# adlternative/adlsm-tree

Measured on AMD Instinct MI355X. Metric: Mkeys/s bloom-filter build (device-resident), 16B keys, bits/key=10, higher is better.
Workload: dtype u32; 1 GPU; 10M x 16B keys, bits_per_key=10, one filter per GPU; keys_per_gpu=10000000, key_bytes=16, bits_per_key=10, filters_per_gpu=1, parallelism=whole filters per GPU x1, no data-path collective

## Files before the change

adlsm-tree_amd/csrc/bloom_build.hip:

```cpp
#include <hip/hip_ext.h>
#include <hip/hip_runtime.h>
#include <stdint.h>
#include <stdlib.h>
#include <string.h>

#include <algorithm>
#include <atomic>
#include <cmath>
#include <mutex>
#include <type_traits>
#include <vector>

#include "bloom_common.hpp"
#include "probe_server.hpp"

using namespace adl_dev;

namespace {

constexpr uint32_t kLdsWordsPerCu = 40960;
constexpr int kKptMax = 8;
constexpr int kBlockB = 1024;
constexpr int kDepthB = 8;
constexpr int kSegBatch = 2048;
// ... 316 lines not shown
        for (uint32_t win = 0; win < nwin; ++win) {
          const uint64_t wb = A0 + (uint64_t)win * S;
          const uint64_t we = min(wb + wcap, B1);
          const uint32_t nv = (uint32_t)((we - wb) >> 4);
          const uint4 *src = reinterpret_cast<const uint4 *>(keys.keys + wb);
          for (uint32_t v = tid; v < nv; v += BLOCK) stage4[v] = src[v];
          const uint32_t rem = (uint32_t)(we - wb) & 15u;
          if (rem && (uint32_t)tid < rem)
            reinterpret_cast<uint8_t *>(lpos)[nv * 16 + tid] = keys.keys[wb + nv * 16 + tid];
          __syncthreads();
          STAMP(6);
          const uint32_t wlo = win * S;
#pragma unroll
          for (int i = 0; i < KPT; ++i) {
            if (ks0[i] - wlo < S) {
              hash_lds(lpos, ks0[i] - wlo, klen[i], h1[i], h2[i]);
              pending &= ~(1u << i);
            }
          }
          __syncthreads();
          STAMP(7);
        }
#pragma unroll
        for (int i = 0; i < KPT; ++i)
          if (pending & (1u << i)) keys.hash(kb + kidx[i], h1[i], h2[i]);
      } else {
#pragma unroll
        for (int i = 0; i < KPT; ++i) {
          h1[i] = h2[i] = 0;
          if (slot_pos(i) < cnt) keys.hash(d.key_begin + first + kidx[i], h1[i], h2[i]);
        }
      }
    } else {
#pragma unroll
      for (int i = 0; i < KPT; ++i) {
        h1[i] = h2[i] = 0;
        if (slot_pos(i) < cnt) {
          if constexpr (PF) hash16(cur[i].raw, h1[i], h2[i]);
          else keys.hash(d.key_begin + first + kidx[i], h1[i], h2[i]);
        }
      }
    }
    uint32_t live = 0;
#pragma unroll
    for (int i = 0; i < KPT; ++i) {
      if (slot_pos(i) < cnt) {
        const uint32_t ki = first + kidx[i];
        if (!(a.dedup && ki > 0 && keys.same_as_prev(d.key_begin + ki))) live |= 1u << i;
      }
    }
    __syncthreads();
    STAMP(1);

    constexpr int KR = KFIX > 0 ? KFIX : 1;
    uint32_t pos[KPT][KR];
#pragma unroll
    for (int i = 0; i < KPT; ++i) {
      if (live & (1u << i)) {
        if constexpr (KFIX > 0) {
#pragma unroll
          for (int j = 0; j < KFIX; ++j) {
            pos[i][j] = fastmod(h1[i] + (uint32_t)j * h2[i], mod);
            atomicAdd(&hist[pos[i][j] >> TL], 1u);
          }
        } else {
          for (uint32_t j = 0; j < k; ++j) {
            const uint32_t p = fastmod(h1[i] + j * h2[i], mod);
            atomicAdd(&hist[p >> TL], 1u);
          }
        }
      }
    }
    __syncthreads();
    STAMP(2);

    const uint32_t total = block_excl_scan_array_1b<BLOCK>(hist, T + 1, scratch);

    uint32_t *tab = table_ws + d.table_base;
    for (uint32_t t = tid; t <= T; t += BLOCK) tab[(uint64_t)t * d.chunks + w] = hist[t];
    __syncthreads();
    STAMP(3);

#pragma unroll
    for (int i = 0; i < KPT; ++i) {
      if (live & (1u << i)) {
        if constexpr (KFIX > 0) {
          uint32_t slot_l[KFIX];
#pragma unroll
          for (int j = 0; j < KFIX; ++j) slot_l[j] = atomicAdd(&hist[pos[i][j] >> TL], 1u);
#pragma unroll
          for (int j = 0; j < KFIX; ++j) lpos[slot_l[j]] = pos[i][j] & tmask;
        } else {
          for (uint32_t j = 0; j < k; ++j) {
            const uint32_t p = fastmod(h1[i] + j * h2[i], mod);
            const uint32_t slot_l = atomicAdd(&hist[p >> TL], 1u);
            lpos[slot_l] = p & tmask;
          }
        }
      }
    }
    __syncthreads();
    STAMP(4);

    for (uint32_t i = tid; i <= T; i += BLOCK) hist[i] = 0;
    uint32_t *dst = pos_ws + d.pos_base + (uint64_t)w * a.cap;
    const uint32_t nvec = total >> 2;
    const uint4 *src4 = reinterpret_cast<const uint4 *>(lpos);
    uint4 *dst4 = reinterpret_cast<uint4 *>(dst);
    for (uint32_t i = tid; i < nvec; i += BLOCK) dst4[i] = src4[i];
    for (uint32_t i = (nvec << 2) + tid; i < total; i += BLOCK) dst[i] = lpos[i];
    STAMP(5);

    if constexpr (PF) {
#pragma unroll
      for (int i = 0; i < KPT; ++i) cur[i] = nxt[i];
    }
  }
  STAMP_FLUSH(0);
}

#ifndef ADL_HV_BLOCK
#define ADL_HV_BLOCK 256
#endif
constexpr int kHvBlock = ADL_HV_BLOCK;
constexpr uint32_t kHvBins = 512;
template <uint32_t S>
constexpr uint32_t hv_stage_bytes() {
  return S * 48;
}

template <uint32_t S>
constexpr size_t hv_lds_bytes() {
  return kHvBins * 4 + S * 4 + S * 2 + hv_stage_bytes<S>() + 16;
}

template <uint32_t S, bool DT>
__global__ __launch_bounds__(kHvBlock) void hash_var_kernel(BuildArgs a, KeysVar keys, uint2 *__restrict__ hp,
                                                            uint32_t total_sc, FilterTable ft) {
  extern __shared__ __attribute__((aligned(16))) uint32_t lds[];
  uint32_t *bins = lds;
  uint32_t *s_rel = lds + kHvBins;
  uint16_t *s_len = reinterpret_cast<uint16_t *>(s_rel + S);
  uint32_t *stage = reinterpret_cast<uint32_t *>(s_len + S);
  constexpr int KPT = S / kHvBlock;
  constexpr uint32_t NW = kHvBlock / kWave;
  const int tid = threadIdx.x, lane = tid & (kWave - 1), wave = tid / kWave;
  const uint32_t sc = blockIdx.x;
  if (sc >= total_sc) return;
  STAMP_DECL
  const auto &d = Filt<DT>::at(a, ft, Filt<DT>::of_run(a, ft, sc));
  const uint32_t first = (sc - d.sc_base) * S;
  const uint32_t cnt = min(S, d.n - first);
  const uint64_t kb = d.key_begin + first;
  const uint64_t base16 = keys.offs[kb] & ~15ull;
  const uint64_t end = keys.offs[kb + cnt];
  constexpr uint32_t kStage = hv_stage_bytes<S>();
  static_assert(kStage % (16 * kHvBlock) == 0, "the staging loads cover kStage in whole rounds of 16 B per thread");
  const uint32_t sbytes = (uint32_t)min((end - base16 + 15) & ~15ull, (uint64_t)kStage);

  constexpr int VPT = kStage / 16 / kHvBlock;
  const uint32_t nv = sbytes / 16;
  for (uint32_t i = tid; i < kHvBins; i += kHvBlock) bins[i] = 0;
  uint64_t o0[KPT], o1[KPT];
#pragma unroll
  for (int i = 0; i < KPT; ++i) {
    const uint32_t idx = min((uint32_t)(tid + i * kHvBlock), cnt - 1u);
    o0[i] = keys.offs[kb + idx];
    o1[i] = keys.offs[kb + idx + 1];
  }
  u32x4_t v[VPT];
  if (nv) {
    const u32x4_t *src = reinterpret_cast<const u32x4_t *>(keys.keys + base16);
#pragma unroll
    for (int i = 0; i < VPT; ++i) v[i] = src[min((uint32_t)(tid + i * kHvBlock), nv - 1u)];
  }
  __syncthreads();
  STAMP(0);
  uint32_t rk[KPT];
#pragma unroll
  for (int i = 0; i < KPT; ++i) {
    rk[i] = ~0u;
    if (tid + i * kHvBlock < cnt) {
      const uint32_t c = (uint32_t)min(o1[i] - o0[i], (uint64_t)(kHvBins - 1));
      rk[i] = (atomicAdd(&bins[c], 1u) << 9) | c;
    }
  }
  {
    u32x4_t *dst = reinterpret_cast<u32x4_t *>(stage);
#pragma unroll
    for (int i = 0; i < VPT; ++i)
      if (tid + i * kHvBlock < nv) dst[tid + i * kHvBlock] = v[i];
  }
  __syncthreads();
  STAMP(1);
  if (wave == 0) {
    constexpr int PER = kHvBins / kWave;
    uint32_t bv[PER], t = 0;
#pragma unroll
    for (int j = 0; j < PER; ++j) bv[j] = bins[lane * PER + j], t += bv[j];
    uint32_t run = wave_incl_scan(t, lane) - t;
#pragma unroll
    for (int j = 0; j < PER; ++j) bins[lane * PER + j] = run, run += bv[j];
  }
  __syncthreads();
  STAMP(2);
#pragma unroll
  for (int i = 0; i < KPT; ++i) {
    if (rk[i] != ~0u) {
      const uint32_t slot = bins[rk[i] & (kHvBins - 1)] + (rk[i] >> 9);
      const uint64_t len = o1[i] - o0[i];
      const bool near = len < 0xffffu && o0[i] - base16 < 0xffffffffull;
      s_rel[slot] = near ? (uint32_t)(o0[i] - base16) : tid + i * kHvBlock;
      s_len[slot] = near ? (uint16_t)len : (uint16_t)0xffffu;
    }
  }
  __syncthreads();
  STAMP(3);

  const uint32_t groups = (cnt + kWave - 1) / kWave;
  uint2 *out = hp + (uint64_t)d.chunk_base * a.C + first;
  for (uint32_t gi = wave; gi < groups; gi += NW) {
    const uint32_t g = groups - 1 - gi;
    const uint32_t s = g * kWave + lane;
    if (s >= cnt) continue;
    uint32_t len = s_len[s];
    const uint32_t r = s_rel[s];
    uint32_t h1, h2;
#ifdef ADL_BLOOM_STAMPS
    if (a.exp & 16) {
      out[s] = make_uint2(r, len | 1u);
      continue;
    }
#endif
    if (len < 0xffffu && (uint64_t)r + len <= sbytes) {
      hash_lds(stage, r, len, h1, h2);
    } else {
      uint64_t k0 = base16 + r;
      if (len == 0xffffu) {
        k0 = keys.offs[kb + r];
        len = (uint32_t)(keys.offs[kb + r + 1] - k0);
      }
      hash_bytes(keys.keys + k0, len, kSeed1, kSeed2, h1, h2);
    }
    out[s] = make_uint2(h1, h2);
  }
  STAMP(4);
  STAMP_FLUSH(2);
}

struct Src16 {
  const uint4 *keys;
  using Raw = uint4;
  __device__ __forceinline__ Raw load(const FilterDesc &d, uint32_t chunk, uint32_t first, uint32_t idx) const {
    return load_nt(keys + d.key_begin + first + idx);
  }
  __device__ static __forceinline__ void hash(const Raw &r, uint32_t &h1, uint32_t &h2) { hash16(r, h1, h2); }
};

typedef uint32_t u32x2_t __attribute__((ext_vector_type(2)));
struct SrcH {
  const uint2 *h;
  uint32_t C;
  using Raw = uint2;
  __device__ __forceinline__ Raw load(const FilterDesc &, uint32_t chunk, uint32_t, uint32_t idx) const {
    const u32x2_t v = __builtin_nontemporal_load(reinterpret_cast<const u32x2_t *>(h + (uint64_t)chunk * C + idx));
    return make_uint2(v.x, v.y);
  }
  __device__ static __forceinline__ void hash(const Raw &r, uint32_t &h1, uint32_t &h2) {
    h1 = r.x;
    h2 = r.y;
  }
};

template <int BLOCK, int K, class Src, bool DT, bool CL = false, bool DYN = false>
__global__ __launch_bounds__(BLOCK) kPassARegs void bloom_bin16_kernel(BuildArgs a, Src keys,
                                                              uint32_t *__restrict__ pos_ws,
                                                              uint32_t *__restrict__ table_ws,
                                                              uint32_t total_chunks, uint32_t *__restrict__ scratch_ws,
                                                              FilterTable ft) {
  using FT = Filt<DT>;
  constexpr int KPT = 6;
  constexpr int VPT = (K * KPT + 3) / 4;
  constexpr int SPI = (VPT + KPT - 1) / KPT;
  extern __shared__ __attribute__((aligned(16))) uint32_t lds[];
  const int tid = threadIdx.x;
  const uint32_t C = a.C;
  const uint32_t TL = a.TL;
  const uint32_t tmask = (1u << TL) - 1u;
  uint32_t *hist = lds;
  uint32_t *scratch = lds + a.hist_words;
  uint32_t *lpos = lds + a.hist_words + 32;
  const uint4 *src4 = reinterpret_cast<const uint4 *>(lpos);
  uint32_t *hist2 = lpos + a.cap;
  uint32_t *oflag = hist2 + a.hist_words;
  uint32_t *after = CL ? oflag + 4 : lpos + K * C;

  const uint32_t G = gridDim.x;
  const uint32_t slot = G % 8 == 0 ? (blockIdx.x % 8) * (G / 8) + blockIdx.x / 8 : blockIdx.x;

  const int wave = tid / kWave;
  uint32_t *dummy = scratch_ws + kQueueWords + ((uint64_t)blockIdx.x * (BLOCK / kWave) + wave) * 4;
  uint4 *dummy4 = reinterpret_cast<uint4 *>(dummy);
  constexpr int TPT = (int)((kHistMax + BLOCK - 1) / BLOCK);

  using Raw = typename Src::Raw;
  auto fetch = [&](uint32_t chunk, Raw (&raw)[KPT]) {
    const auto &d = FT::at(a, ft, FT::of_chunk(a, ft, chunk));
    const uint32_t first = (chunk - d.chunk_base) * C;
    const uint32_t last = min(C, d.n - first) - 1u;
#pragma unroll
    for (int i = 0; i < KPT; ++i) {
      const uint32_t idx = min((uint32_t)(tid + i * BLOCK), last);
      raw[i] = keys.load(d, chunk, first, idx);
    }
  };

  Raw raw[KPT];
  uint32_t h1[KPT], h2[KPT];
  uint32_t wg0 = slot, n1 = slot + G, n2 = slot + 2 * G;
  uint32_t *qa = lds + (a.hist_words + 28);
  [[maybe_unused]] GroupQueue gq(scratch_ws, G, total_chunks);
  if constexpr (DYN) {
    if (tid == 0) {
      qa[0] = gq.next();
      qa[1] = gq.next();
      qa[2] = gq.next();
    }
    __syncthreads();
    wg0 = qa[0];
    n1 = qa[1];
    n2 = qa[2];
    __syncthreads();
  }
  if (wg0 >= total_chunks) return;
  fetch(wg0, raw);
#pragma unroll
  for (int i = 0; i < KPT; ++i) Src::hash(raw[i], h1[i], h2[i]);
  fetch(min(n1, total_chunks - 1), raw);
  for (uint32_t i = tid; i < a.hist_words; i += BLOCK) hist[i] = 0;
  if constexpr (CL)
    for (uint32_t i = tid; i < a.hist_words + 4; i += BLOCK) hist2[i] = 0;

  const uint32_t dd = a.dd_log2;
  uint32_t *dtab32 = after;
  if (dd)
    for (uint32_t i = tid; i < (2u << dd); i += BLOCK) dtab32[i] = ~0u;

  uint4 *pdst = dummy4;
  uint32_t ptotal = 0;
  uint32_t par = 0;
  uint32_t qpar = 0;
  STAMP_DECL
  for (uint32_t wg = wg0; wg < total_chunks;) {
    [[maybe_unused]] uint32_t n3 = 0;
    if (DYN && tid == 0) n3 = gq.next();
    const int fcur = FT::of_chunk(a, ft, wg);
    const auto &d = FT::at(a, ft, fcur);
    const uint32_t w = wg - d.chunk_base;
    const uint32_t cnt = min(C, d.n - w * C);
    const uint32_t T = d.tiles;
    const FastMod mod = d.mod;
    uint32_t *hcur = hist, *hoth = hist2;
    if (CL && par) hcur = hist2, hoth = hist;
    const uint32_t tcap = CL ? (a.cap / T) & ~3u : 0u;
    __syncthreads();
    STAMP(0);

    const uint32_t pvec = ptotal >> 2;
    uint32_t live = 0;
#pragma unroll
    for (int i = 0; i < KPT; ++i)
      if (tid + i * BLOCK < cnt) live |= 1u << i;
    if (dd) {
      uint32_t old[KPT];
#pragma unroll
      for (int i = 0; i < KPT; ++i) {
        const uint32_t sl = h1[i] >> (31 - dd);
        old[i] = ((live >> i) & 1u) && h1[i] == h2[i] ? atomicCAS(&dtab32[sl], ~0u, h1[i]) : ~0u;
      }
#pragma unroll
      for (int i = 0; i < KPT; ++i)
        if (old[i] != ~0u && old[i] == h1[i] && h1[i] == h2[i]) live &= ~(1u << i);
    }
    uint32_t pos[KPT][K];
#pragma unroll
    for (int i = 0; i < KPT; ++i) {
      if ((live >> i) & 1u) {
#pragma unroll
        for (int j = 0; j < K; ++j) pos[i][j] = fastmod(h1[i] + (uint32_t)j * h2[i], mod);
#ifdef ADL_BLOOM_STAMPS
        if (a.exp & 32)
#pragma unroll
          for (int j = 0; j < K; ++j) pos[i][j] = (h1[i] + (uint32_t)j * h2[i]) >> 3;
#endif
#ifdef ADL_BLOOM_STAMPS
        if (a.exp & 64)
#pragma unroll
          for (int j = 0; j < K; ++j)
            pos[i][j] = (((uint32_t)(tid & 63) + (i == 0 && j == 0 && tid < 64 ? 64u : 0u)) << TL) | (pos[i][j] & tmask);
#endif
        if constexpr (!CL)
#pragma unroll
          for (int j = 0; j < K; ++j) atomicAdd(&hist[pos[i][j] >> TL], 1u);
      }
      if constexpr (!CL) {
#pragma unroll
        for (int sv = i * SPI; sv < (i + 1) * SPI && sv < VPT; ++sv) {
          const uint32_t v = tid + sv * BLOCK;
          bool ok = v < pvec;
#ifdef ADL_BLOOM_STAMPS
          if (a.exp & 2) ok = false;
#endif
          *(ok ? pdst + v : dummy4) = src4[ok ? v : 0u];
        }
      }
    }
    if constexpr (!CL) {
      const bool ok = (uint32_t)tid < (ptotal & 3u);
      *(ok ? reinterpret_cast<uint32_t *>(pdst) + pvec * 4 + tid : dummy) = lpos[ok ? pvec * 4 + tid : 0u];
    }
    uint32_t *tab = table_ws + d.table_base;
    uint32_t total = 0;
    if constexpr (!CL) {
      __syncthreads();
      STAMP(1);

      total = block_excl_scan_array_1b<BLOCK>(hist, T + 1, scratch);
      STAMP(2);
#pragma unroll
      for (int r = 0; r < TPT; ++r) {
        const uint32_t t = tid + r * BLOCK;
        const bool ok = t <= T;
        *(ok ? tab + (uint64_t)t * d.chunks + w : dummy) = hist[ok ? t : 0u];
      }
      __syncthreads();
      STAMP(3);
    }

    bool ovf = false;
#pragma unroll
    for (int i = 0; i < KPT; ++i) {
      if ((live >> i) & 1u) {
        uint32_t sl[K];
        if constexpr (CL) {
#pragma unroll
          for (int j = 0; j < K; ++j) sl[j] = atomicAdd(&hcur[pos[i][j] >> TL], 1u);
#pragma unroll
          for (int j = 0; j < K; ++j) {
            if (sl[j] < tcap) lpos[(pos[i][j] >> TL) * tcap + sl[j]] = pos[i][j] & tmask;
            else ovf = true;
          }
        } else {
#pragma unroll
          for (int j = 0; j < K; ++j) sl[j] = atomicAdd(&hist[pos[i][j] >> TL], 1u);
#pragma unroll
          for (int j = 0; j < K; ++j) lpos[sl[j]] = pos[i][j] & tmask;
        }
      }
#ifdef ADL_BLOOM_STAMPS
      if (a.exp & 1) {
        h1[i] = raw[i].x;
        h2[i] = raw[i].y | 1u;
      } else
#endif
        Src::hash(raw[i], h1[i], h2[i]);
    }
    fetch(min(n2, total_chunks - 1), raw);
    const bool last_of_filter = n1 >= total_chunks || FT::of_chunk(a, ft, n1) != fcur;
    if (CL && ovf) oflag[par] = 1u;
    if (DYN && tid == 0) qa[qpar] = n3;
    __syncthreads();
    STAMP(4);
    if constexpr (CL) {
      for (uint32_t i = tid; i < a.hist_words; i += BLOCK) hoth[i] = 0;
      if (tid == 0) oflag[par ^ 1u] = 0;
    } else {
      for (uint32_t i = tid; i <= T; i += BLOCK) hist[i] = 0;
    }
    if (dd && last_of_filter && n1 < total_chunks)
      for (uint32_t i = tid; i < (2u << dd); i += BLOCK) dtab32[i] = ~0u;
    if constexpr (CL) {
      uint4 *dst = reinterpret_cast<uint4 *>(pos_ws + d.pos_base + (uint64_t)w * a.cap);
      if (oflag[par] == 0u) {
#pragma unroll
        for (int r = 0; r < TPT; ++r) {
          const uint32_t t = tid + r * BLOCK;
          const bool ok = t < T;
          *(ok ? tab + (uint64_t)t * d.chunks + w : dummy) = ((t * tcap) << 16) | hcur[ok ? t : 0u];
        }
        const uint32_t tq = tcap >> 2, nvec = T * tq;
        const uint32_t mg = 0xffffffffu / tq + 1u;
#pragma unroll
        for (int sv = 0; sv < VPT; ++sv) {
          const uint32_t v = tid + sv * BLOCK;
          const uint32_t t = __umulhi(v, mg);
          const bool ok = v < nvec && 4u * (v - t * tq) < hcur[min(t, T - 1u)];
          *(ok ? dst + v : dummy4) = src4[ok ? v : 0u];
        }
      } else {
        total = block_excl_scan_array<BLOCK>(hcur, T + 1, scratch);
#pragma unroll
        for (int r = 0; r < TPT; ++r) {
          const uint32_t t = tid + r * BLOCK;
          const bool ok = t < T;
          const uint32_t s0 = hcur[ok ? t : 0u], s1 = hcur[ok ? t + 1 : 0u];
          *(ok ? tab + (uint64_t)t * d.chunks + w : dummy) = (s0 << 16) | (s1 - s0);
        }
        __syncthreads();
#pragma unroll
        for (int i = 0; i < KPT; ++i) {
          if ((live >> i) & 1u) {
            uint32_t sl[K];
#pragma unroll
            for (int j = 0; j < K; ++j) sl[j] = atomicAdd(&hcur[pos[i][j] >> TL], 1u);
#pragma unroll
            for (int j = 0; j < K; ++j) lpos[sl[j]] = pos[i][j] & tmask;
          }
        }
        __syncthreads();
        const uint32_t tv = total >> 2;
#pragma unroll
        for (int sv = 0; sv < VPT; ++sv) {
          const uint32_t v = tid + sv * BLOCK;
          const bool ok = v < tv;
          *(ok ? dst + v : dummy4) = src4[ok ? v : 0u];
        }
        const bool ok = (uint32_t)tid < (total & 3u);
        *(ok ? reinterpret_cast<uint32_t *>(dst) + tv * 4 + tid : dummy) = lpos[ok ? tv * 4 + tid : 0u];
      }
      par ^= 1u;
    } else {
      pdst = reinterpret_cast<uint4 *>(pos_ws + d.pos_base + (uint64_t)w * a.cap);
      ptotal = total;
    }
    wg = n1;
    n1 = n2;
    if constexpr (DYN) {
      n2 = qa[qpar];
      qpar ^= 1u;
    } else {
      n2 += G;
    }
  }
  const uint32_t pvec = ptotal >> 2;
  for (uint32_t v = tid; v < pvec; v += BLOCK) pdst[v] = src4[v];
  if ((uint32_t)tid < (ptotal & 3u))
    reinterpret_cast<uint32_t *>(pdst)[pvec * 4 + tid] = lpos[pvec * 4 + tid];
  STAMP(5);
  STAMP_FLUSH(0);
}

template <int D, bool DT, int OCC = 1, bool DYN = false, int BLK = kBlockB>
__global__ __launch_bounds__(BLK, 4 * OCC) void bloom_tile_kernel(BuildArgs a,
                                                             const uint32_t *__restrict__ pos_ws,
                                                             const uint32_t *__restrict__ table_ws,
                                                             uint8_t *__restrict__ bitmaps,
                                                             uint32_t total_tiles, uint32_t *__restrict__ scratch_ws,
                                                             FilterTable ft) {
  using FT = Filt<DT>;
  extern __shared__ __attribute__((aligned(16))) uint32_t lds[];
  const int tid = threadIdx.x, lane = tid & (kWave - 1), wave = tid / kWave;
  constexpr int NWAVES = BLK / kWave;
  constexpr int SEGB = OCC == 2 ? BLK : 2 * BLK;
  static_assert(SEGB <= kSegBatch, "the plan's LDS holds kSegBatch descriptors");
  constexpr int RPT = SEGB / BLK;
  const uint32_t TL = a.TL;
  const uint32_t tile_words = 1u << (TL - 5);
  if (blockIdx.x == 0 && tid == 0) scratch_ws[kLayoutWord] = a.claim ? kLayoutClaim : kLayoutDense;
  uint32_t *tile = lds;
  uint2 *seg = reinterpret_cast<uint2 *>(lds + tile_words);
  uint32_t *qb = lds + tile_words + 2 * SEGB;

  auto fetch_rows = [&](uint32_t wg, uint32_t wb, uint32_t (&rs)[RPT], uint32_t (&re)[RPT]) {
    const auto &d = FT::at(a, ft, FT::of_tile(a, ft, wg));
    const uint32_t lt = wg - d.tile_base, W = d.chunks;
    const uint32_t *row0 = table_ws + d.table_base + (uint64_t)lt * W;
#pragma unroll
    for (int r = 0; r < RPT; ++r) {
      const uint32_t i = wb + tid + r * BLK;
      rs[r] = re[r] = 0;
      if (i < W) {
        if (a.claim) {
          const uint32_t v = row0[i];
          rs[r] = v >> 16;
          re[r] = rs[r] + (v & 0xffffu);
        } else {
          rs[r] = row0[i];
          re[r] = row0[i + W];
        }
      }
    }
  };
#ifdef ADL_BLOOM_STAMPS
  uint32_t exp_sink = 0;
  auto or_pos = [&](uint32_t off) {
    if (a.exp & 4) exp_sink += off;
    else atomicOr(&tile[off >> 5], 1u << (off & 31));
  };
#else
  auto or_pos = [&](uint32_t off) { atomicOr(&tile[off >> 5], 1u << (off & 31)); };
#endif

  const uint32_t G = gridDim.x;
  uint32_t wg = G % 8 == 0 ? (blockIdx.x % 8) * (G / 8) + blockIdx.x / 8 : blockIdx.x;
  uint32_t nxt = wg + G;
  [[maybe_unused]] GroupQueue gq(scratch_ws + 8 * 16, G, total_tiles);
  uint32_t qpar = 0;
  if constexpr (DYN) {
    if (tid == 0) {
      qb[0] = gq.next();
      qb[1] = gq.next();
    }
    __syncthreads();
    wg = qb[0];
    nxt = qb[1];
    __syncthreads();
  }
  uint32_t pre_s[RPT], pre_e[RPT];
  if (wg < total_tiles) fetch_rows(wg, 0, pre_s, pre_e);
  {
    uint4 *t4w = reinterpret_cast<uint4 *>(tile);
    for (uint32_t i = tid; i < tile_words / 4; i += BLK) t4w[i] = make_uint4(0, 0, 0, 0);
  }
  STAMP_DECL

  while (wg < total_tiles) {
    const int fi = FT::of_tile(a, ft, wg);
    const auto &d = FT::at(a, ft, fi);
    const uint32_t lt = wg - d.tile_base;
    const uint32_t W = d.chunks;
    const uint32_t pos_base = (uint32_t)d.pos_base;
    STAMP(0);
    const uint32_t next = nxt;
    [[maybe_unused]] uint32_t nn = 0;
    if (DYN && tid == 0) nn = gq.next();
    if (W == 0 && next < total_tiles) fetch_rows(next, 0, pre_s, pre_e);

    for (uint32_t wb = 0; wb < W; wb += SEGB) {
      const uint32_t nw = min((uint32_t)SEGB, W - wb);
      uint32_t rs[RPT], re[RPT];
      if (wb == 0) {
#pragma unroll
        for (int r = 0; r < RPT; ++r) rs[r] = pre_s[r], re[r] = pre_e[r];
      } else {
        fetch_rows(wg, wb, rs, re);
      }
#pragma unroll
      for (int r = 0; r < RPT; ++r) {
        const uint32_t i = tid + r * BLK;
        if (i < nw) seg[i] = make_uint2(pos_base + (wb + i) * a.cap + rs[r], re[r] - rs[r]);
      }
      __syncthreads();
      STAMP(1);
      if (wb + SEGB >= W && next < total_tiles) fetch_rows(next, 0, pre_s, pre_e);

      const uint32_t Q = nw > (uint32_t)wave ? (nw - wave + NWAVES - 1) / NWAVES : 0;
      struct Stage {
        uint32_t v0[D], v1[D];
        uint32_t base, len;
      };
      auto issue = [&](Stage &st, uint32_t q0) {
        const uint32_t q = q0 + lane;
        uint2 dsc = make_uint2(0, 0);
        if (lane < D && q < Q) dsc = seg[wave + NWAVES * q];
        st.base = dsc.x;
        st.len = dsc.y;
        uint32_t len[D];
        const uint32_t *sp[D];
#pragma unroll
        for (int u = 0; u < D; ++u) {
          len[u] = __builtin_amdgcn_readlane(st.len, u);
          sp[u] = pos_ws + __builtin_amdgcn_readlane(st.base, u);
        }
#pragma unroll
        for (int u = 0; u < D; ++u)
          if (len[u] > (uint32_t)kWave && (uint32_t)lane + kWave < len[u]) st.v1[u] = sp[u][kWave + lane];
#pragma unroll
        for (int u = 0; u < D; ++u) st.v0[u] = sp[u][lane];
      };
      auto consume = [&](const Stage &st) {
#pragma unroll
        for (int u = 0; u < D; ++u) {
          const uint32_t len = __builtin_amdgcn_readlane(st.len, u);
          if ((uint32_t)lane < len) or_pos(st.v0[u]);
          if (len > (uint32_t)kWave) {
            if ((uint32_t)lane + kWave < len) or_pos(st.v1[u]);
            if (len > 2u * kWave) {
              const uint32_t b = __builtin_amdgcn_readlane(st.base, u);
              for (uint32_t o = 2 * kWave; o < len; o += 4 * kWave) {
                uint32_t x[4];
#pragma unroll
                for (int t = 0; t < 4; ++t) {
                  const uint32_t e = o + t * kWave + lane;
                  x[t] = e < len ? pos_ws[b + e] : 0u;
                }
#pragma unroll
                for (int t = 0; t < 4; ++t)
                  if (o + t * kWave + lane < len) or_pos(x[t]);
              }
            }
          }
        }
      };
      Stage A, B;
      issue(A, 0);
      for (uint32_t q0 = 0; q0 < Q; q0 += 2 * D) {
        issue(B, q0 + D);
        consume(A);
        issue(A, q0 + 2 * D);
        consume(B);
      }
      __syncthreads();
      STAMP(2);
    }

    const uint64_t tile_bytes = 1ull << (TL - 3);
    const uint64_t b0 = (uint64_t)lt * tile_bytes;
    const uint64_t nbytes = min(tile_bytes, (uint64_t)d.alloc_bytes - b0);
    uint4 *out4 = reinterpret_cast<uint4 *>(bitmaps + d.bitmap_off + b0);
    const uint4 *t4 = reinterpret_cast<const uint4 *>(tile);
    uint4 *t4z = reinterpret_cast<uint4 *>(tile);
    const uint32_t nvec = (uint32_t)(nbytes >> 4);
    for (uint32_t i = tid; i < tile_words / 4; i += BLK) {
      const uint4 v = t4[i];
      t4z[i] = make_uint4(0, 0, 0, 0);
      if (i < nvec) {
#ifdef ADL_BLOOM_STAMPS
        if (a.exp & 8) continue;
#endif
        store_nt(out4 + i, v);
      }
    }
    if (DYN && tid == 0) qb[qpar] = nn;
    __syncthreads();
    STAMP(3);
    wg = next;
    if constexpr (DYN) {
      nxt = qb[qpar];
      qpar ^= 1u;
    } else {
      nxt = next + G;
    }
  }
#ifdef ADL_BLOOM_STAMPS
  if (exp_sink == 0x9e3779b9u) scratch_ws[kQueueWords] = exp_sink;
#endif
  STAMP_FLUSH(1);
}

struct Plan {
  BuildArgs a;
  std::vector<FilterDesc> f;
  bool dt = false;
  uint64_t pos_words = 0, table_words = 0, scratch_words = 0, hash_words = 0, ft_bytes = 0, ws_bytes = 0;
  bool claim = false;
  uint32_t total_chunks = 0, total_tiles = 0, total_sc = 0;
  uint32_t grid_a = 0, grid_b = 0;
  uint32_t occ_b = 1;
  size_t lds_a = 0, lds_b = 0;
};

int make_plan(const uint64_t *counts, uint32_t nf, int32_t bpk, Plan &p) {
  if (nf == 0 || bpk < 0) return ADL_ERR_INVALID_ARG;
  const adl_host::Knobs &kn = adl_host::knobs();
  memset(&p.a, 0, sizeof(p.a));
  p.f.assign(nf, FilterDesc{});
  p.dt = nf > (uint32_t)kMaxFilters;
  const uint32_t k = (uint32_t)adl_host::num_probes(bpk);
// ... 583 lines not shown
```

Before: 64460 Mkeys/s.

## Stagger hash/scatter order across wave groups and batch LDS-to-global copies

Waves are split into two roles by wave index: one group hashes all next-chunk keys before doing its LDS atomic scatter, the other interleaves scatter and hash per slot. The aim is to de-synchronise LDS atomic traffic across waves so ALU hashing overlaps other waves' LDS contention. The LDS-to-global position copy is restructured to issue all loads before the stores, and hashing is skipped when there is no next chunk. It adds code duplication and register pressure from the split paths and the buffered uint4 values.

```diff
diff --git a/adlsm-tree_amd/csrc/bloom_build.hip b/adlsm-tree_amd/csrc/bloom_build.hip
--- a/adlsm-tree_amd/csrc/bloom_build.hip
+++ b/adlsm-tree_amd/csrc/bloom_build.hip
@@ -642,6 +642,7 @@
   uint32_t *dummy = scratch_ws + kQueueWords + ((uint64_t)blockIdx.x * (BLOCK / kWave) + wave) * 4;
   uint4 *dummy4 = reinterpret_cast<uint4 *>(dummy);
   constexpr int TPT = (int)((kHistMax + BLOCK - 1) / BLOCK);
+  const bool role1 = (__builtin_amdgcn_readfirstlane(wave) >> 2) & 1;
 
   using Raw = typename Src::Raw;
   auto fetch = [&](uint32_t chunk, Raw (&raw)[KPT]) {
@@ -703,6 +704,7 @@
     uint32_t *hcur = hist, *hoth = hist2;
     if (CL && par) hcur = hist2, hoth = hist;
     const uint32_t tcap = CL ? (a.cap / T) & ~3u : 0u;
+    const bool hash_next = n1 < total_chunks;
     __syncthreads();
     STAMP(0);
 
@@ -744,15 +746,20 @@
           for (int j = 0; j < K; ++j) atomicAdd(&hist[pos[i][j] >> TL], 1u);
       }
       if constexpr (!CL) {
-#pragma unroll
-        for (int sv = i * SPI; sv < (i + 1) * SPI && sv < VPT; ++sv) {
-          const uint32_t v = tid + sv * BLOCK;
-          bool ok = v < pvec;
+        uint4 q[SPI];
+        bool ok[SPI];
+#pragma unroll
+        for (int s = 0; s < SPI; ++s) {
+          const uint32_t v = tid + (i * SPI + s) * BLOCK;
+          ok[s] = i * SPI + s < VPT && v < pvec;
 #ifdef ADL_BLOOM_STAMPS
-          if (a.exp & 2) ok = false;
+          if (a.exp & 2) ok[s] = false;
 #endif
-          *(ok ? pdst + v : dummy4) = src4[ok ? v : 0u];
+          if (i * SPI + s < VPT) q[s] = src4[ok[s] ? v : 0u];
         }
+#pragma unroll
+        for (int s = 0; s < SPI; ++s)
+          if (i * SPI + s < VPT) *(ok[s] ? pdst + (tid + (i * SPI + s) * BLOCK) : dummy4) = q[s];
       }
     }
     if constexpr (!CL) {
@@ -778,8 +785,7 @@
     }
 
     bool ovf = false;
-#pragma unroll
-    for (int i = 0; i < KPT; ++i) {
+    auto scatter_slot = [&](int i) {
       if ((live >> i) & 1u) {
         uint32_t sl[K];
         if constexpr (CL) {
@@ -797,6 +803,9 @@
           for (int j = 0; j < K; ++j) lpos[sl[j]] = pos[i][j] & tmask;
         }
       }
+    };
+    auto hash_slot = [&](int i) {
+      if (!hash_next) return;
 #ifdef ADL_BLOOM_STAMPS
       if (a.exp & 1) {
         h1[i] = raw[i].x;
@@ -804,6 +813,18 @@
       } else
 #endif
         Src::hash(raw[i], h1[i], h2[i]);
+    };
+    if (role1) {
+#pragma unroll
+      for (int i = 0; i < KPT; ++i) hash_slot(i);
+#pragma unroll
+      for (int i = 0; i < KPT; ++i) scatter_slot(i);
+    } else {
+#pragma unroll
+      for (int i = 0; i < KPT; ++i) {
+        scatter_slot(i);
+        hash_slot(i);
+      }
     }
     fetch(min(n2, total_chunks - 1), raw);
     const bool last_of_filter = n1 >= total_chunks || FT::of_chunk(a, ft, n1) != fcur;
```

New measurement: 64790 Mkeys/s, median of 6. No clear change (+0.5%).
